# EnnaDelfen/SUHMO

Hardware: AMD Instinct MI355X
Metric: multigrid V-cycles/s (FAS head solve) + GSRB cell-updates/s; achieved HBM GB/s vs peak (higher is better)
Workload: dtype f64; 1 GPU; SHMIP-A head solve, 4096x4096 cells per GPU (square cells of 24.4 m), single AMR level, 64x64 boxes, 6 MG depths, 4+4 GSRB sweeps per depth, 16 bottom (BASELINE north_star: 4096^2 single-level); partition=none

## Files before the change

### suhmo_amd/csrc/suhmo_common.h

```cpp
#pragma once
#include <hip/hip_runtime.h>
#include <cstdio>
#include <cstdlib>
#include <cstring>
#include <utility>
#include <string>
#include <vector>
#include "../../include/suhmo_hip.h"

#define SUHMO_XOFF 16
#define SUHMO_MAXDEPTH 16

struct DV {
    int nx, ny;
    int P;
    int gy;
    int rows;
    int j0, nyg;
    double dx, dy;
    double rdx, rdy;
    double fdx, fdy;
    double alpha, beta;
    int bct[2][2];
    double two_v[2][2];
// ... 112 lines not shown
    int poll_readback;
    size_t scratch_elems;
    suhmo_exchange_fn ex;
    suhmo_allreduce_max_fn ar;
    suhmo_allreduce_fn ar2;
    int (*ard)(void *user, double *dev_values, int n, int op, suhmo_stream_t s);
    void *user;
    int (*ex_begin)(void *user);
    int (*ex_end)(void *user, suhmo_level *L, suhmo_stream_t s);
    long graph_max_cells;
    std::vector<VGraph> vgraphs; int vgraph_seen[4]; hipStream_t gstream;
    suhmo_level *gap; double gap_dt;
    void *rccl;
    int faces_deferred;
    void *ipc; int ipc_owner;
    long agg_min_cells;
    int agg_depth, agg_world, agg_rank;
    suhmo_level *agg;
    int agg_static_stale;
    suhmo_allgather_fn ag; void *ag_user;
    double *agg_send, *agg_recv; size_t agg_cap; long agg_gathers;
    int resout_req, resout_armed, resout_done; const double *resout_rhs; long resout_count;
    int resout_np;
    long frhs_stream, frhs_tile;
    int prof_on;
    std::vector<ProfEv> prof;
    int gsrb_variant;
    long fused_min_cells;
    int bcoef_fused;
    int bcoef_tile_x;
    int fused_nt;
    int fused_restrict;
    int fused_hc;
    int fas_rhs_fused;
    int strips_rhs_local;
    int skip_mask;
    int mask_reported;
    int coarse_mask_ok;
    unsigned mask_epoch, maskflag_epoch;
    int overlap_halo;
    hipStream_t xstream; hipEvent_t xev[2]; long overlapped;
    int tile_strips;
    int tile_chunks;
    int resid_in_relax;
    int fas_rhs_in_relax;
    long tile_max_cells;
    int tile_restrict;
    int tile_order;
    int bottom_solver; long bottom_one_launch_max_cells;
    unsigned long long *bottom_ctr; long bottom_host_iters, bottom_host_solves;
    int gsrb_tile, tile_t, tile_s;
};

void suhmo_set_error(const char *fmt, ...);
struct SuhmoTimer { const char *name; double t0; int mode; explicit SuhmoTimer(const char *n); ~SuhmoTimer(); };
#define SUHMO_TIME(label) SuhmoTimer suhmo_tm_(label)
#define HIPCHK(x) do { hipError_t e_ = (x); if (e_ != hipSuccess) { \
    suhmo_set_error("%s:%d %s -> %s", __FILE__, __LINE__, #x, hipGetErrorString(e_)); return -2; } } while (0)
#define ARG(cond) do { if (!(cond)) { suhmo_set_error("%s:%d bad argument: %s", __FILE__, __LINE__, #cond); return -1; } } while (0)

double *suhmo_field(suhmo_level *L, int depth, int field);
int suhmo_level_create_(suhmo_level_t **out, const suhmo_level_desc_t *desc, bool stub);
void suhmo_level_share_transport(suhmo_level *dst, const suhmo_level *src);
int suhmo_level_materialize_(suhmo_level *L);
void suhmo_fp_changed();
unsigned long suhmo_fp_epoch();
// ... 66 lines not shown
```

### suhmo_amd/csrc/suhmo_gsrb.hip

```cpp
#include "suhmo_hier.h"
#include <type_traits>

template <bool HAS_ALPHA>
__device__ __forceinline__ void d_gsrb_pass_simple(const DV &v, const FP &fp, suhmo_phys_t ph, int pass, int jlo, int jhi,
                                                   const FP *__restrict__ ft = nullptr, const int2 *__restrict__ push = nullptr)
{
    int j = jlo + (int)(blockIdx.y * blockDim.y + threadIdx.y);
    int t = blockIdx.x * blockDim.x + threadIdx.x;
    if (j > jhi) return;
    int i = 2 * t + ((j + v.j0 + pass) & 1);
    if (i >= v.nx) return;
    double *__restrict__ phi = fp.f[SUHMO_F_PHI];
    int idx = cidx(v, i, j);
    double c = phi[idx];
    double e = phiE(v, phi, idx, i, c, false), w = phiW(v, phi, idx, i, c, false);
    double n = phiN(v, phi, idx, j, c, false), s = phiS(v, phi, idx, j, c, false);
    double bxW = fp.f[SUHMO_F_BX][idx], bxE = fp.f[SUHMO_F_BX][idx + 1];
    double byS = fp.f[SUHMO_F_BY][idx], byN = fp.f[SUHMO_F_BY][idx + v.P];
    double nl, dnl;
    nl_terms(ph, c, fp.f[SUHMO_F_B][idx], fp.f[SUHMO_F_PI][idx], fp.f[SUHMO_F_ZB][idx],
             fp.f[SUHMO_F_MASK][idx], nl, dnl);
    double aterm = HAS_ALPHA ? v.alpha * fp.f[SUHMO_F_ACOEF][idx] : v.alpha;
    double lofphi = lofphi_cell(v, aterm, c, e, w, n, s, bxE, bxW, byN, byS, nl);
    double lam = lambda_cell(v, aterm, bxE, bxW, byN, byS);
// ... 202 lines not shown
    const dim3 grd(((m.maxnx + T - 1) / T) * ((m.maxny + T - 1) / T), m.nbox);
    if (has_alpha) hipLaunchKernelGGL((k_gsrb_box_m<true, G, T, S>), grd, dim3(BoxGeom<G, T, S>::NT), 0, st, m.dv, m.fp, (const int2 *)halo, hbase, ph, fsrc, fdst, npass, bc_ghosts);
    else hipLaunchKernelGGL((k_gsrb_box_m<false, G, T, S>), grd, dim3(BoxGeom<G, T, S>::NT), 0, st, m.dv, m.fp, (const int2 *)halo, hbase, ph, fsrc, fdst, npass, bc_ghosts);
}
int suhmo_multi_gsrb_box(const suhmo_multi &m, const suhmo_phys_t &ph, bool has_alpha, const void *halo, const int *hbase, int fsrc, int fdst, int npass, int bc_ghosts, hipStream_t st)
{
    if (m.nbox <= 0) return 0;
    if (npass < 1 || npass > 2 * SUHMO_BOX_HALO) { suhmo_set_error("internal: %d colour passes in one box launch", npass); return -4; }
    if (npass > 4) launch_box<8, 16, 1>(m, ph, has_alpha, halo, hbase, fsrc, fdst, npass, bc_ghosts, st);
    else launch_box<4, 16, 1>(m, ph, has_alpha, halo, hbase, fsrc, fdst, npass, bc_ghosts, st);
    HIPCHK(hipGetLastError());
    return 0;
}

struct FusedGeom {
    int W;
    int Hc;
    int nstrips, nchunks, ntiles;
    int ylo, yhi;
    int jbeg, jend;
    int wrap_y;
    const unsigned *negflag; unsigned mask_epoch;
    int nchl, chunk0, chunk1, edges;
    const double *pc, *pco; int Pc, gyc;
    double *rres, *rphi; int rP, rgy;
    const double *fres; double *frhs, *flphi, *fphiold;
    const double *ortrue; double *ores, *olphi;
    double *onorm;
};

struct RowCoef {
    double rhs[2], B[2], Pi[2], zb[2], mask[2], a[2], byS[2], byN[2];
    double bx0, bx1, bx2;
};
#define CP2(d, s, f) d.f[0] = s.f[0]; d.f[1] = s.f[1]
template <bool HAS_ALPHA>
__device__ __forceinline__ void copy_coef(RowCoef &d, const RowCoef &s)
{
    CP2(d, s, rhs); CP2(d, s, B); CP2(d, s, Pi); CP2(d, s, zb); CP2(d, s, mask);
    if (HAS_ALPHA) { CP2(d, s, a); }
    CP2(d, s, byS); CP2(d, s, byN);
    d.bx0 = s.bx0; d.bx1 = s.bx1; d.bx2 = s.bx2;
}

template <int K, bool HAS_ALPHA, int NT, int RM = 0, bool FRHS = false>
__global__ __launch_bounds__(NT) void k_gsrb_fused(DV v, FP fp, const double *__restrict__ pin,
                                                   double *__restrict__ pout, suhmo_phys_t ph, FusedGeom g)
{
    constexpr bool ROUT = RM == 2, RR = RM != 0;
    static_assert(!(FRHS && (RR || HAS_ALPHA)), "the right-hand side is formed in the plain launch of an alpha = 0 operator");
    constexpr int LW = 2 * NT, R = 2 * K + 3 + (RR ? 1 : 0);
    constexpr int HX = 2 * K + (RR ? 2 : 0), EY = RR ? 1 : 0;
    __shared__ double lds[R * LW];

    int b = blockIdx.x, q = g.ntiles / 8, rem = g.ntiles % 8, xcd = b % 8;
    int tile = xcd * q + (xcd < rem ? xcd : rem) + b / 8;
    int strip = tile / g.nchl, chunk = tile % g.nchl;
    chunk = g.edges ? (chunk < g.chunk0 ? chunk : g.chunk1 + (chunk - g.chunk0)) : g.chunk0 + chunk;

    const int t = threadIdx.x;
    const int c0 = strip * g.W;
    const int xl = 2 * t;
    const int i0 = c0 - HX + xl;
    const bool in_row = xl < g.W + 2 * HX;
    int im = i0;
    if (v.per[0]) { if (im < 0) im += v.nx; else if (im >= v.nx) im -= v.nx; }
    const bool cval = in_row && im >= 0 && im < v.nx;
    const int cend = (c0 + g.W < v.nx) ? c0 + g.W : v.nx;
    const bool own = cval && i0 >= c0 && i0 < cend;

    const int jA = g.jbeg + chunk * g.Hc;
    const int jB = (jA + g.Hc < g.jend) ? jA + g.Hc : g.jend;
    const int jmin = (jA - EY - 2 * K > g.ylo) ? jA - EY - 2 * K : g.ylo;
    const int jmax = (jB - 1 + EY + 2 * K < g.yhi) ? jB - 1 + EY + 2 * K : g.yhi;

    const double *__restrict__ f_rhs = fp.f[SUHMO_F_RHS], *__restrict__ f_B = fp.f[SUHMO_F_B];
    const double *__restrict__ f_Pi = fp.f[SUHMO_F_PI], *__restrict__ f_zb = fp.f[SUHMO_F_ZB];
    const double *__restrict__ f_mask = fp.f[SUHMO_F_MASK], *__restrict__ f_a = fp.f[SUHMO_F_ACOEF];
    const double *__restrict__ f_bx = fp.f[SUHMO_F_BX], *__restrict__ f_by = fp.f[SUHMO_F_BY];

    auto wrapj = [&](int j) { if (g.wrap_y) { if (j < 0) j += v.ny; else if (j >= v.ny) j -= v.ny; } return j; };
    auto ld2 = [&](const double *__restrict__ p, int idx) { return *reinterpret_cast<const double2 *>(p + idx); };

    RowCoef cf0, cf1, cf2, cf3, cf4, cf5;
    double racc = 0.0, raccp = 0.0;
    double nmax = 0.0;
    const bool xbc = !v.per[0] && (c0 - HX <= 0 || c0 + g.W + HX >= v.nx);
    const bool ybc = !v.per[1] && (jmin <= 0 || jmax >= v.ny - 1);
    double2 pnext = make_double2(0.0, 0.0);
    double2 pprev = make_double2(0.0, 0.0);
    const bool usemask = !g.negflag || *g.negflag == g.mask_epoch;

    int sr = 0;
    auto ring = [](int x) { return x < 0 ? x + R : x; };
    for (int r = jmin - 1; r <= jB - 1 + 2 * K + EY; r++) {
        bool lphi = cval && (r + 1 >= jmin) && (r + 1 <= jmax);
        if (lphi) {
            const int jr = wrapj(r + 1);
            pnext = ld2(pin, cidx(v, im, jr));
            if (g.pc) {
                const int ic = ((jr >> 1) + g.gyc) * g.Pc + SUHMO_XOFF + (im >> 1);
                const double corr = 1.0 * g.pc[ic] + (-1.0) * g.pco[ic];
                pnext.x = pnext.x + corr; pnext.y = pnext.y + corr;
            }
        }
        bool lcf = cval && (r >= jmin) && (r <= jmax);
        if (lcf) {
            int idx = cidx(v, im, wrapj(r));
#define LD2(dst, p, ix) { double2 t_ = ld2(p, ix); dst[0] = t_.x; dst[1] = t_.y; }
            LD2(cf0.rhs, (FRHS ? g.fres : f_rhs), idx); LD2(cf0.B, f_B, idx); LD2(cf0.Pi, f_Pi, idx);
            LD2(cf0.zb, f_zb, idx);
            if (usemask) { LD2(cf0.mask, f_mask, idx); } else { cf0.mask[0] = 1.0; cf0.mask[1] = 1.0; }
            if (HAS_ALPHA) LD2(cf0.a, f_a, idx);
            LD2(cf0.byS, f_by, idx); LD2(cf0.byN, f_by, idx + v.P);
            double2 bxp = ld2(f_bx, idx);
            cf0.bx0 = bxp.x; cf0.bx1 = bxp.y; cf0.bx2 = f_bx[idx + 2];
        }
        __syncthreads();

        if constexpr (FRHS) {
            const int jf = r - 1;
            if (cval && jf >= jmin && jf <= jmax) {
                const int s0 = ring(sr - 1), sN = sr;
                const double *row = lds + s0 * LW;
                double lo[2], cc[2];
#pragma unroll
                for (int a = 0; a < 2; a++) {
                    const int x = xl + a, i = im + a;
                    double c = row[x];
                    double w = row[(a == 0 && xl == 0) ? 0 : x - 1], e = row[(a == 1 && xl == LW - 2) ? LW - 1 : x + 1];
                    double n = lds[sN * LW + x], s = a ? pprev.y : pprev.x;
                    if (xbc) {
                        if (i == 0) w = (v.bct[0][0] == 0) ? v.two_v[0][0] - c : c + v.neu[0][0];
                        if (i == v.nx - 1) e = (v.bct[0][1] == 0) ? v.two_v[0][1] - c : c + v.neu[0][1];
                    }
                    if (ybc) {
                        if (jf == 0 && !v.ext[0]) s = (v.bct[1][0] == 0) ? v.two_v[1][0] - c : c + v.neu[1][0];
                        if (jf == v.ny - 1 && !v.ext[1]) n = (v.bct[1][1] == 0) ? v.two_v[1][1] - c : c + v.neu[1][1];
                    }
                    double nl, dnl;
                    nl_terms(ph, c, cf1.B[a], cf1.Pi[a], cf1.zb[a], cf1.mask[a], nl, dnl);
                    const double bxW = a ? cf1.bx1 : cf1.bx0, bxE = a ? cf1.bx2 : cf1.bx1;
                    lo[a] = lofphi_cell(v, v.alpha, c, e, w, n, s, bxE, bxW, cf1.byN[a], cf1.byS[a], nl);
                    cc[a] = c;
                }
                cf1.rhs[0] = 1.0 * cf1.rhs[0] + 1.0 * lo[0]; cf1.rhs[1] = 1.0 * cf1.rhs[1] + 1.0 * lo[1];
                const bool lo_end = v.ext[0] && chunk == 0, hi_end = v.ext[1] && chunk == g.nchunks - 1;
                const int jP0 = lo_end ? jmin : jA, jP1 = hi_end ? jmax + 1 : jB;
                const int jR0 = lo_end ? jmin + 1 : jA, jR1 = hi_end ? jmax : jB;
                if (own && jf >= jP0 && jf < jP1) {
                    const int idx = cidx(v, i0, jf);
                    if (jf >= jR0 && jf < jR1) {
                        *reinterpret_cast<double2 *>(g.flphi + idx) = make_double2(lo[0], lo[1]);
                        *reinterpret_cast<double2 *>(g.frhs + idx) = make_double2(cf1.rhs[0], cf1.rhs[1]);
                    }
                    *reinterpret_cast<double2 *>(g.fphiold + idx) = make_double2(cc[0], cc[1]);
                }
                pprev = make_double2(cc[0], cc[1]);
            }
            __syncthreads();
        }

        auto advance_a = [&](const int m, const RowCoef &q, auto a_tag) {
            constexpr int a = decltype(a_tag)::value;
            const int j = r - m;
            const int x = xl + a, i = im + a;
            const int s0 = ring(sr - m), sN = ring(sr - m + 1), sS = ring(sr - m - 1);
            const double *row = lds + s0 * LW;
            double c = row[x];
            double w = row[(a == 0 && xl == 0) ? 0 : x - 1], e = row[(a == 1 && xl == LW - 2) ? LW - 1 : x + 1];
            double n = lds[sN * LW + x], s = lds[sS * LW + x];
            if (xbc) {
                if (i == 0) w = (v.bct[0][0] == 0) ? v.two_v[0][0] - c : c + v.neu[0][0];
                if (i == v.nx - 1) e = (v.bct[0][1] == 0) ? v.two_v[0][1] - c : c + v.neu[0][1];
            }
            if (ybc) {
                if (j == 0 && !v.ext[0]) s = (v.bct[1][0] == 0) ? v.two_v[1][0] - c : c + v.neu[1][0];
                if (j == v.ny - 1 && !v.ext[1]) n = (v.bct[1][1] == 0) ? v.two_v[1][1] - c : c + v.neu[1][1];
            }
            double nl, dnl;
            nl_terms(ph, c, q.B[a], q.Pi[a], q.zb[a], q.mask[a], nl, dnl);
            const double bxW = a ? q.bx1 : q.bx0, bxE = a ? q.bx2 : q.bx1;
            double aterm = HAS_ALPHA ? v.alpha * q.a[a] : v.alpha;
            double lofphi = lofphi_cell(v, aterm, c, e, w, n, s, bxE, bxW, q.byN[a], q.byS[a], nl);
            double lam = lambda_cell(v, aterm, bxE, bxW, q.byN[a], q.byS[a]);
            double denom = 1.0e-16 + lam + dnl;
            lds[s0 * LW + x] = c + (q.rhs[a] - lofphi) / denom;
        };
        auto advance = [&](const int m, const RowCoef &q) {
            const int j = r - m;
            if (j >= jmin && j <= jmax) {
                const int a = (j + v.j0 + ((m - 1) & 1)) & 1;
                if (a) { if (cval) advance_a(m, q, std::integral_constant<int, 1>()); }
                else   { if (cval) advance_a(m, q, std::integral_constant<int, 0>()); }
            }
        };
        advance(1, cf1);
        __syncthreads();
        advance(2, cf2);
        if constexpr (K >= 2) {
            __syncthreads();
            advance(3, cf3);
            __syncthreads();
            advance(4, cf4);
        }

        if constexpr (RR) {
            const int jr = r - 2 * K - 1;
            if (own && jr >= jA && jr < jB && jr >= 0 && jr < v.ny) {
                const RowCoef &q = (K >= 2) ? cf5 : cf3;
                const int s0 = ring(sr - (2 * K + 1)), sN = ring(sr - 2 * K), sS = ring(sr - (2 * K + 2));
                const double *row = lds + s0 * LW;
                double acc = (jr & 1) ? racc : 0.0, accp = (jr & 1) ? raccp : 0.0;
                double lo2[2] = {0.0, 0.0};
#pragma unroll
                for (int a = 0; a < 2; a++) {
                    const int x = xl + a, i = im + a;
                    double c = row[x], w = row[x - 1], e = row[x + 1];
                    double n = lds[sN * LW + x], s = lds[sS * LW + x];
                    if (xbc) {
                        if (i == 0) w = (v.bct[0][0] == 0) ? v.two_v[0][0] - c : c + v.neu[0][0];
                        if (i == v.nx - 1) e = (v.bct[0][1] == 0) ? v.two_v[0][1] - c : c + v.neu[0][1];
                    }
                    if (ybc) {
                        if (jr == 0 && !v.ext[0]) s = (v.bct[1][0] == 0) ? v.two_v[1][0] - c : c + v.neu[1][0];
                        if (jr == v.ny - 1 && !v.ext[1]) n = (v.bct[1][1] == 0) ? v.two_v[1][1] - c : c + v.neu[1][1];
                    }
                    double nl, dnl;
                    nl_terms(ph, c, q.B[a], q.Pi[a], q.zb[a], q.mask[a], nl, dnl);
                    const double bxW = a ? q.bx1 : q.bx0, bxE = a ? q.bx2 : q.bx1;
                    double aterm = HAS_ALPHA ? v.alpha * q.a[a] : v.alpha;
                    double lofphi = lofphi_cell(v, aterm, c, e, w, n, s, bxE, bxW, q.byN[a], q.byS[a], nl);
                    if constexpr (ROUT) lo2[a] = lofphi;
                    else {
                        acc = acc + (q.rhs[a] - lofphi) / 4.0;
                        accp = accp + c / 4.0;
                    }
                }
                if constexpr (ROUT) {
                    const int idx = cidx(v, i0, jr);
                    const double2 rt = *reinterpret_cast<const double2 *>(g.ortrue + idx);
                    const double r0 = -1.0 * lo2[0] + 1.0 * rt.x, r1 = -1.0 * lo2[1] + 1.0 * rt.y;
                    *reinterpret_cast<double2 *>(g.ores + idx) = make_double2(r0, r1);
                    if (g.olphi) *reinterpret_cast<double2 *>(g.olphi + idx) = make_double2(lo2[0], lo2[1]);
                    nmax = fmax(nmax, fmax(fabs(r0), fabs(r1)));
                } else if (jr & 1) {
                    const int ic = ((jr >> 1) + g.rgy) * g.rP + SUHMO_XOFF + (i0 >> 1);
                    g.rres[ic] = acc; g.rphi[ic] = accp;
                } else { racc = acc; raccp = accp; }
            }
        }
        {
            const int jo = r - 2 * K;
            if (own && jo >= jA && jo < jB) {
                const int so = ring(sr - 2 * K);
                double2 o = make_double2(lds[so * LW + xl], lds[so * LW + xl + 1]);
                *reinterpret_cast<double2 *>(pout + cidx(v, i0, jo)) = o;
            }
        }
        sr = sr + 1 == R ? 0 : sr + 1;
        if (in_row) { lds[sr * LW + xl] = pnext.x; lds[sr * LW + xl + 1] = pnext.y; }
        if constexpr (RR && K >= 2) copy_coef<HAS_ALPHA>(cf5, cf4);
        if constexpr (K >= 2) { copy_coef<HAS_ALPHA>(cf4, cf3); copy_coef<HAS_ALPHA>(cf3, cf2); }
        else if constexpr (RR) copy_coef<HAS_ALPHA>(cf3, cf2);
        copy_coef<HAS_ALPHA>(cf2, cf1);
        copy_coef<HAS_ALPHA>(cf1, cf0);
    }
    if constexpr (ROUT) {
        if (g.onorm) {
            static_assert(!ROUT || NT == 64, "one wave per workgroup");
#pragma unroll
            for (int o = 32; o > 0; o >>= 1) nmax = fmax(nmax, __shfl_xor(nmax, o));
            if (t == 0) g.onorm[strip * g.nchunks + chunk] = nmax;
        }
    }
}

static bool fused_ok(const suhmo_level *L, const Depth &D, int K)
{
    const DV &v = D.v;
    if (v.nx % 2 || v.nx < 64 || v.ny < 4 * K + 4) return false;
    if (v.cfx[0] || v.cfx[1] || L->desc.nx_global > 0) return false;
    if ((v.ext[0] || v.ext[1]) && (v.gy < 2 * K || v.ny < 2 * K)) return false;
    if (v.per[1] && !(v.ext[0] || v.ext[1]) && v.ny < 4 * K) return false;
    return true;
}

template <int K, int NT, int RM = 0>
static int launch_fused(suhmo_level *L, int depth, int ext_rows, hipStream_t st, int part = 0)
{
    constexpr bool RST = RM == 1, RR = RM != 0;
    Depth &D = L->d[depth];
    const DV &v = D.v;
    if (!D.phi_alt) {
        HIPCHK(hipMalloc(&D.phi_alt, D.elems * sizeof(double)));
        HIPCHK(hipMemsetAsync(D.phi_alt, 0, D.elems * sizeof(double), st));
    }
    FusedGeom g;
    constexpr int HX = 2 * K + (RR ? 2 : 0), EY = RR ? 1 : 0;
// ... 48 lines not shown
    g.negflag = nullptr; g.mask_epoch = 0;
    if (L->skip_mask && L->maskflag_epoch && L->maskflag_epoch == L->mask_epoch && (depth == 0 || L->coarse_mask_ok)
        && (L->desc.nx_global == 0)) {
        g.negflag = (const unsigned *)(L->scratch + L->scratch_elems - 1); g.mask_epoch = L->mask_epoch;
    }
    g.rres = g.rphi = nullptr; g.rP = g.rgy = 0;
    if (RST) {
        Depth &C = L->d[depth + 1];
        g.rres = C.fp.f[SUHMO_F_RES]; g.rphi = C.fp.f[SUHMO_F_PHI]; g.rP = C.v.P; g.rgy = C.v.gy;
        C.phi_fresh = 0;
    }
    g.fres = nullptr; g.frhs = g.flphi = g.fphiold = nullptr;
    g.ortrue = nullptr; g.ores = g.olphi = nullptr;
    if (RM == 2) {
        if (v.alpha != 0.0) { suhmo_set_error("internal: residual output on a launch that cannot form it"); return -4; }
        g.ortrue = L->resout_rhs ? L->resout_rhs : D.fp.f[SUHMO_F_RHS];
        g.ores = D.fp.f[SUHMO_F_RES];
        if (L->resout_req & 2) { g.olphi = suhmo_field(L, depth, SUHMO_F_LPHI); if (!g.olphi) return -2; }
        g.onorm = nullptr;
        if ((L->resout_req & 4) && (size_t)g.nstrips * g.nchunks + 4 < L->scratch_elems) { g.onorm = L->scratch + 2; L->resout_np = g.nstrips * g.nchunks; }
        else L->resout_np = 0;
    }
    if (D.rhs_pending) {
        if constexpr (K == 2 && NT == 64 && !RR) {
            if (part || v.alpha != 0.0) { suhmo_set_error("internal: rhs_pending on a launch that cannot form it"); return -4; }
            g.fres = D.fp.f[SUHMO_F_RES]; g.frhs = D.fp.f[SUHMO_F_RHS]; g.flphi = suhmo_field(L, depth, SUHMO_F_LPHI); g.fphiold = suhmo_field(L, depth, SUHMO_F_PHIOLD);
            if (!g.flphi || !g.fphiold) return -2;
            D.rhs_pending = 0; L->frhs_stream++;
            hipLaunchKernelGGL((k_gsrb_fused<2, false, 64, false, true>), dim3(g.ntiles), dim3(NT), 0, st, v, D.fp, pin, D.phi_alt, L->ph, g);
            { std::swap(D.fp.f[SUHMO_F_PHI], D.phi_alt); suhmo_fp_changed(); }
            return 0;
        } else { suhmo_set_error("internal: rhs_pending on a launch that cannot form it"); return -4; }
    }
    if (v.alpha != 0.0)
        hipLaunchKernelGGL((k_gsrb_fused<K, true, NT, false>), dim3(g.ntiles), dim3(NT), 0, st, v, D.fp, pin, D.phi_alt, L->ph, g);
    else
        hipLaunchKernelGGL((k_gsrb_fused<K, false, NT, RM>), dim3(g.ntiles), dim3(NT), 0, st, v, D.fp, pin, D.phi_alt, L->ph, g);
    if (part != 1) { std::swap(D.fp.f[SUHMO_F_PHI], D.phi_alt); suhmo_fp_changed(); }
    return 0;
}

struct TileGeom {
    int ntx, nty;
    const double *pc, *pco; int Pc, gyc;
    double *rres, *rphi; int rP, rgy;
    int frhs;
    int jbeg, jend;
    int chunks;
    int order;
};
struct PairCoef { double rhs0, rhs1, B0, B1, Pi0, Pi1, zb0, zb1, a0, a1, byS0, byS1, byN0, byN1, bx0, bx1, bx2; int mneg; };

template <int T, bool RST> struct TileShape { static constexpr int TX = T, TY = (RST && T == 32) ? 28 : T; };
template <int S, int T, bool RST> struct TileThreads { static constexpr int NT = 256; };
template <int S, int T, bool HAS_ALPHA, bool RST = false, bool CHUNKED = false>
__global__ __launch_bounds__((TileThreads<S, T, RST>::NT)) __attribute__((amdgpu_waves_per_eu((TileThreads<S, T, RST>::NT == 384 ? 3 : 2)))) void k_gsrb_tile(DV v,
    FP fp, const double *__restrict__ pin, double *__restrict__ pout,
                                                   suhmo_phys_t ph, TileGeom g)
{
    constexpr int TX = TileShape<T, RST>::TX, TY = TileShape<T, RST>::TY;
    constexpr int HX = 2 * S + (RST ? 2 : 0), HY = 2 * S + (RST ? 1 : 0);
    constexpr int LX = TX + 2 * HX, LY = TY + 2 * HY, NP = LX / 2, NPAIR = NP * LY;
    constexpr int NT = TileThreads<S, T, RST>::NT, NK = (NPAIR + NT - 1) / NT;
    constexpr int PAD = LX + 2;
    __shared__ double lds_raw[LY * LX + 2 * PAD];
    double *const lds = lds_raw + PAD;
    __shared__ double lq[RST ? TY * TX : 1];
    int tl = blockIdx.x;
    if (g.order) {
// ... 560 lines not shown
```

### suhmo_amd/csrc/suhmo_level.hip

```cpp
#include "suhmo_hier.h"
#include "suhmo_level_int.h"
#include <algorithm>
#include <cstdarg>
#include <cmath>
#include <initializer_list>

static thread_local char g_err[512] = "";
void suhmo_set_error(const char *fmt, ...)
{
    va_list ap; va_start(ap, fmt); vsnprintf(g_err, sizeof(g_err), fmt, ap); va_end(ap);
}
extern "C" const char *suhmo_last_error(void) { return g_err; }
#include <atomic>
#include <chrono>
#include <map>
#include <mutex>
namespace {
std::atomic<int> g_timer_mode{-1};
std::mutex g_timer_mu;
struct TimerRec { long count = 0; double total = 0.0; };
std::map<std::string, TimerRec> g_timers;
inline double now_s() { return std::chrono::duration<double>(std::chrono::steady_clock::now().time_since_epoch()).count(); }
inline int timer_mode()
{
// ... 108 lines not shown
{
    ARG(out && desc);
    ARG(desc->nx >= 2 && desc->ny >= 2 && desc->dx > 0 && desc->dy > 0);
    ARG(desc->ny_global >= desc->ny && desc->j0 >= 0 && desc->j0 + desc->ny <= desc->ny_global);
    ARG(desc->i0 >= 0 && (desc->nx_global == 0 ? desc->i0 == 0 : desc->i0 + desc->nx <= desc->nx_global));
    ARG(desc->i0 % 2 == 0);
    ARG(desc->patch_ny == 0 || (desc->nx_global > 0 && desc->patch_j0 <= desc->j0 && desc->j0 + desc->ny <= desc->patch_j0 + desc->patch_ny));
    ARG((long)(desc->nx + 64) * (long)(desc->ny + 2 * (desc->halo_rows < 1 ? 1 : desc->halo_rows)) < (1L << 31));
    int ndev = 0;
    HIPCHK(hipGetDeviceCount(&ndev));
    if (ndev <= 0) { suhmo_set_error("no HIP device: the product path has no CPU fallback"); return -3; }
    ARG(desc->device >= 0 && desc->device < ndev);
    HIPCHK(hipSetDevice(desc->device));
    suhmo_level *L = new suhmo_level();
    L->desc = *desc; L->ph = desc->phys; L->device = desc->device;
    L->ex = nullptr; L->ar = nullptr; L->ar2 = nullptr; L->ard = nullptr; L->user = nullptr; L->ex_begin = nullptr; L->ex_end = nullptr; L->rccl = nullptr;
        L->ipc = nullptr; L->ipc_owner = 0; L->faces_deferred = 0; L->gap = nullptr; L->gap_dt = 0.0; L->prof_on = 0; L->gsrb_variant = -1; L->fused_hc = 0;
    L->bcoef_fused = 1;
    L->bcoef_tile_x = 62;
    L->fused_nt = 64;
    L->fused_restrict = 1;
    L->gsrb_tile = 1; L->tile_t = 0; L->tile_s = 4;
    L->tile_max_cells = 3000000;
    L->fas_rhs_in_relax = 3;
    L->tile_chunks = 1;
    L->tile_order = 2; L->tile_restrict = 0;
    L->tile_strips = 1;
    L->overlap_halo = 1; L->xstream = nullptr; L->xev[0] = L->xev[1] = nullptr; L->overlapped = 0;
    L->strips_rhs_local = 1;
    L->fas_rhs_fused = 1;
    L->agg_min_cells = 100000; L->agg_depth = 0; L->agg_world = 1; L->agg_rank = 0; L->agg = nullptr; L->ag = nullptr; L->ag_user = nullptr;
    L->agg_send = L->agg_recv = nullptr; L->agg_cap = 0; L->agg_gathers = 0; L->agg_static_stale = 0;
    L->frhs_stream = L->frhs_tile = 0;
    L->resout_np = 0;
    L->resout_req = L->resout_armed = L->resout_done = 0; L->resout_rhs = nullptr; L->resout_count = 0; L->resid_in_relax = 1;
    L->graph_max_cells = 1500000; L->gstream = nullptr; memset(L->vgraph_seen, 0, sizeof(L->vgraph_seen));
    L->fused_min_cells = 1000000;
    L->skip_mask = 1; L->poll_readback = 1;
    L->bottom_solver = 0; L->bottom_one_launch_max_cells = 16384;
    L->bottom_ctr = nullptr; L->bottom_host_iters = L->bottom_host_solves = 0;
    {
        struct IntKnob { const char *env; int suhmo_level::*field; };
        struct LongKnob { const char *env; long suhmo_level::*field; };
        static const IntKnob ints[] = {
            {"SUHMO_GSRB_VARIANT", &suhmo_level::gsrb_variant}, {"SUHMO_FUSED_HC", &suhmo_level::fused_hc}, {"SUHMO_BCOEF_FUSED", &suhmo_level::bcoef_fused},
            {"SUHMO_BCOEF_TILE_X", &suhmo_level::bcoef_tile_x}, {"SUHMO_FUSED_NT", &suhmo_level::fused_nt}, {"SUHMO_OVERLAP_HALO", &suhmo_level::overlap_halo},
            {"SUHMO_STRIPS_RHS_LOCAL", &suhmo_level::strips_rhs_local}, {"SUHMO_FAS_RHS_FUSED", &suhmo_level::fas_rhs_fused},
            {"SUHMO_RESID_IN_RELAX", &suhmo_level::resid_in_relax}, {"SUHMO_TILE_STRIPS", &suhmo_level::tile_strips}, {"SUHMO_TILE_CHUNKS", &suhmo_level::tile_chunks},
            {"SUHMO_TILE_RESTRICT", &suhmo_level::tile_restrict}, {"SUHMO_TILE_ORDER", &suhmo_level::tile_order}, {"SUHMO_FAS_RHS_IN_RELAX", &suhmo_level::fas_rhs_in_relax},
            {"SUHMO_TILE_S", &suhmo_level::tile_s}, {"SUHMO_GSRB_TILE", &suhmo_level::gsrb_tile}, {"SUHMO_TILE_T", &suhmo_level::tile_t},
            {"SUHMO_FUSED_RESTRICT", &suhmo_level::fused_restrict}, {"SUHMO_SKIP_MASK", &suhmo_level::skip_mask}, {"SUHMO_POLL_READBACK", &suhmo_level::poll_readback}};
        static const LongKnob longs[] = {
            {"SUHMO_AGG_MIN_CELLS", &suhmo_level::agg_min_cells}, {"SUHMO_TILE_MAX_CELLS", &suhmo_level::tile_max_cells},
            {"SUHMO_GRAPH_MAX_CELLS", &suhmo_level::graph_max_cells}, {"SUHMO_FUSED_MIN_CELLS", &suhmo_level::fused_min_cells},
            {"SUHMO_BOTTOM_ONE_LAUNCH_MAX_CELLS", &suhmo_level::bottom_one_launch_max_cells}};
        for (const IntKnob &k : ints) if (const char *e = getenv(k.env)) L->*(k.field) = atoi(e);
        for (const LongKnob &k : longs) if (const char *e = getenv(k.env)) L->*(k.field) = atol(e);
        L->fas_rhs_fused = L->fas_rhs_fused != 0;
        if (L->tile_order < 0 || L->tile_order > 2) L->tile_order = 0;
        if (L->tile_t != 16 && L->tile_t != 32) L->tile_t = 0;
    }
    if (desc->boxes && desc->nbox > 0) {
        L->boxes.assign(desc->boxes, desc->boxes + 4 * (size_t)desc->nbox);
    } else {
        int mb = desc->max_box > 0 ? desc->max_box : 64;
        for (int bj = 0; bj * mb < desc->ny; bj++)
            for (int bi = 0; bi * mb < desc->nx; bi++) {
                int lo0 = desc->i0 + bi * mb, lo1 = desc->j0 + bj * mb;
                int hi0 = std::min(lo0 + mb, desc->i0 + desc->nx) - 1, hi1 = std::min(lo1 + mb, desc->j0 + desc->ny) - 1;
                int b[4] = {lo0, lo1, hi0, hi1};
                L->boxes.insert(L->boxes.end(), b, b + 4);
            }
    }
    L->desc.boxes = nullptr;
    L->desc.nbox = (int)(L->boxes.size() / 4);
    {
        long cells = 0;
        for (size_t k = 0; k < L->boxes.size(); k += 4) {
            const int *b = &L->boxes[k];
            if (b[0] < desc->i0 || b[2] >= desc->i0 + desc->nx || b[1] < desc->j0 || b[3] >= desc->j0 + desc->ny || b[0] > b[2] || b[1] > b[3]) {
                suhmo_set_error("box %zu outside the strip", k / 4); delete L; return -1;
            }
            cells += (long)(b[2] - b[0] + 1) * (b[3] - b[1] + 1);
        }
        if (cells != (long)desc->nx * desc->ny) { suhmo_set_error("boxes do not tile the level"); delete L; return -1; }
    }
    L->ndepth = 1;
    for (int dep = 1; dep < SUHMO_MAXDEPTH; dep++) {
        if (!boxes_coarsenable(L->boxes, (1 << dep) * 2)) break;
        if ((desc->j0 % (1 << dep)) || (desc->ny_global % (1 << dep))) break;
        if ((desc->i0 % (2 << dep)) || (desc->nx_global % (1 << dep))) break;
        L->ndepth = dep + 1;
    }
// ... 63 lines not shown
    for (int dep = 0; dep < L->ndepth; dep++) make_dv(L->d[dep].v, L->desc, dep);
    suhmo_level_drop_graphs(L);
    return 0;
}
extern "C" int suhmo_level_set_alpha_beta(suhmo_level_t *L, double alpha, double beta)
{
    ARG(L);
    L->desc.alpha = alpha; L->desc.beta = beta;
    if (L->agg) { int rc = suhmo_level_set_alpha_beta(L->agg, alpha, beta); if (rc) return rc; }
    return remake_views(L);
}
extern "C" int suhmo_level_set_bc(suhmo_level_t *L, const suhmo_bc_t *bc)
{
    ARG(L && bc);
    for (int d = 0; d < 2; d++)
        if ((bc->periodic[d] != 0) != (L->desc.bc.periodic[d] != 0)) { suhmo_set_error("setBC cannot change the periodicity of the domain"); return -1; }
    for (int d = 0; d < 2; d++) for (int s = 0; s < 2; s++) ARG(bc->type[d][s] == 0 || bc->type[d][s] == 1);
    L->desc.bc = *bc;
    if (L->agg) { int rc = suhmo_level_set_bc(L->agg, bc); if (rc) return rc; }
    return remake_views(L);
}

static long *option_slot_long(suhmo_level *L, const char *key)
{
    if (!strcmp(key, "fused_min_cells")) return &L->fused_min_cells;
    if (!strcmp(key, "tile_max_cells")) return &L->tile_max_cells;
    if (!strcmp(key, "graph_max_cells")) return &L->graph_max_cells;
    if (!strcmp(key, "agg_min_cells")) return &L->agg_min_cells;
    return nullptr;
}
static int *option_slot_int(suhmo_level *L, const char *key)
{
    static const struct { const char *k; int suhmo_level::*m; } tab[] = {
        {"gsrb_variant", &suhmo_level::gsrb_variant}, {"fused_hc", &suhmo_level::fused_hc}, {"bcoef_fused", &suhmo_level::bcoef_fused}, {"bcoef_tile_x", &suhmo_level::bcoef_tile_x},
        {"fused_nt", &suhmo_level::fused_nt}, {"fused_restrict", &suhmo_level::fused_restrict}, {"strips_rhs_local", &suhmo_level::strips_rhs_local},
        {"tile_strips", &suhmo_level::tile_strips}, {"overlap_halo", &suhmo_level::overlap_halo}, {"skip_mask", &suhmo_level::skip_mask}, {"tile_chunks",
            &suhmo_level::tile_chunks}, {"tile_order", &suhmo_level::tile_order}, {"tile_restrict", &suhmo_level::tile_restrict}, {"fas_rhs_in_relax",
            &suhmo_level::fas_rhs_in_relax}, {"resid_in_relax", &suhmo_level::resid_in_relax}, {"fas_rhs_fused", &suhmo_level::fas_rhs_fused},
        {"tile_s", &suhmo_level::tile_s}, {"gsrb_tile", &suhmo_level::gsrb_tile}, {"tile_t", &suhmo_level::tile_t}, {"poll_readback", &suhmo_level::poll_readback}};
    for (const auto &e : tab) if (!strcmp(key, e.k)) return &(L->*(e.m));
    return nullptr;
}
extern "C" int suhmo_level_set_option(suhmo_level_t *L, const char *key, long value)
{
    ARG(L && key);
    if (!strcmp(key, "bottom_solver")) {
        if (value != 0 && value != 1) { suhmo_set_error("bottom_solver: 0 (bottom relaxes only) or 1 (RelaxSolver)"); return -1; }
        return suhmo_bottom_configure(L, (int)value, L->bottom_one_launch_max_cells);
    }
    if (!strcmp(key, "bottom_one_launch_max_cells")) {
        if (value < 0) { suhmo_set_error("bottom_one_launch_max_cells: >= 0"); return -1; }
        return suhmo_bottom_configure(L, L->bottom_solver, value);
    }
    if (long *p = option_slot_long(L, key)) {
        *p = value; suhmo_level_drop_graphs(L);
        if (!strcmp(key, "agg_min_cells")) return suhmo_agg_setup(L);
        return 0;
    }
    if (int *p = option_slot_int(L, key)) {
        if (!strcmp(key, "tile_t") && value != 0 && value != 16 && value != 32) { suhmo_set_error("tile_t: 0 (by size), 16 or 32"); return -1; }
        if (!strcmp(key, "fused_nt") && value != 64 && value != 256) { suhmo_set_error("fused_nt: 64 or 256"); return -1; }
        if (!strcmp(key, "poll_readback") && value && !L->hscratch_dev) { suhmo_set_error("poll_readback: no device address of the host slot"); return -1; }
        *p = (int)value; suhmo_level_drop_graphs(L); return 0;
    }
    suhmo_set_error("unknown option '%s'", key);
    return -1;
}
extern "C" int suhmo_level_get_option(const suhmo_level_t *L, const char *key, long *value)
{
    ARG(L && key && value);
    if (long *p = option_slot_long(const_cast<suhmo_level *>(L), key)) { *value = *p; return 0; }
    if (int *p = option_slot_int(const_cast<suhmo_level *>(L), key)) { *value = *p; return 0; }
    if (!strcmp(key, "overlapped_launches")) { *value = L->overlapped; return 0; }
    if (!strcmp(key, "agg_gathers")) { *value = L->agg_gathers; return 0; }
    if (!strcmp(key, "rhs_in_streaming_launches")) { *value = L->frhs_stream; return 0; }
    if (!strcmp(key, "rhs_in_tile_launches")) { *value = L->frhs_tile; return 0; }
    if (!strcmp(key, "residual_in_relax_launches")) { *value = L->resout_count; return 0; }
    if (!strcmp(key, "bottom_solver")) { *value = L->bottom_solver; return 0; }
    if (!strcmp(key, "bottom_one_launch_max_cells")) { *value = L->bottom_one_launch_max_cells; return 0; }
    if (!strcmp(key, "bottom_solver_iterations")) { *value = suhmo_bottom_counter(L, 0); return 0; }
    if (!strcmp(key, "bottom_solves_one_launch")) { *value = suhmo_bottom_counter(L, 1); return 0; }
    if (!strcmp(key, "bottom_solves_host_loop")) { *value = suhmo_bottom_counter(L, 2); return 0; }
    suhmo_set_error("unknown option '%s'", key);
    return -1;
}

extern "C" int suhmo_level_num_depths(const suhmo_level_t *L) { return L ? L->ndepth : -1; }
extern "C" int suhmo_level_synchronize(suhmo_level_t *L, suhmo_stream_t s)
{
    ARG(L);
    HIPCHK(hipStreamSynchronize((hipStream_t)s));
    return 0;
}
extern "C" int suhmo_level_set_hooks(suhmo_level_t *L, suhmo_exchange_fn ex, suhmo_allreduce_max_fn ar, void *user)
{
    ARG(L);
    L->ex = ex; L->ar = ar; L->ar2 = nullptr; L->ard = nullptr; L->user = user; L->ex_begin = nullptr; L->ex_end = nullptr;
    return 0;
}
void suhmo_level_share_transport(suhmo_level *dst, const suhmo_level *src)
{
    dst->ex = src->ex; dst->ar = src->ar; dst->ar2 = src->ar2; dst->ard = src->ard; dst->user = src->user;
    dst->ex_begin = src->ex_begin; dst->ex_end = src->ex_end; dst->ipc = src->ipc;
}
extern "C" int suhmo_level_set_allgather(suhmo_level_t *L, suhmo_allgather_fn fn, void *user)
{
    ARG(L);
    HIPCHK(hipSetDevice(L->device));
    L->ag = fn; L->ag_user = user;
// ... 228 lines not shown
```

Measured before the change: 487.0 V-cycles/s.

## Add opt-in two-row load prefetch to fused GSRB and trim coefficient registers

Restructures the fused GSRB row loop into issue/step phases so an optional variant can keep loads for two rows in flight, raising memory-level parallelism for the plain alpha=0, K=2, 64-thread launch. The default path also changes: the mask is kept as a sign bitfield, the south face coefficient is reused from the previous row's north face instead of reloaded, and the coarse correction is applied at store time. These changes cut global loads and register pressure, but the mask now enters as ±1, and the two-row path raises register use and is gated behind an option.

Measured after the change: 493.3 V-cycles/s, median of 6. 1.01x the previous value.

```diff
diff --git a/suhmo_amd/csrc/suhmo_common.h b/suhmo_amd/csrc/suhmo_common.h
--- a/suhmo_amd/csrc/suhmo_common.h
+++ b/suhmo_amd/csrc/suhmo_common.h
@@ -168,6 +168,8 @@
     int fused_nt;
     int fused_restrict;
     int fused_hc;
+    int fused_prefetch;
+    long prefetch2_count;
     int fas_rhs_fused;
     int strips_rhs_local;
     int skip_mask;
diff --git a/suhmo_amd/csrc/suhmo_gsrb.hip b/suhmo_amd/csrc/suhmo_gsrb.hip
--- a/suhmo_amd/csrc/suhmo_gsrb.hip
+++ b/suhmo_amd/csrc/suhmo_gsrb.hip
@@ -258,23 +258,35 @@
 struct RowCoef {
     double rhs[2], B[2], Pi[2], zb[2], mask[2], a[2], byS[2], byN[2];
     double bx0, bx1, bx2;
+    int mneg;
 };
 #define CP2(d, s, f) d.f[0] = s.f[0]; d.f[1] = s.f[1]
 template <bool HAS_ALPHA>
 __device__ __forceinline__ void copy_coef(RowCoef &d, const RowCoef &s)
 {
-    CP2(d, s, rhs); CP2(d, s, B); CP2(d, s, Pi); CP2(d, s, zb); CP2(d, s, mask);
+    CP2(d, s, rhs); CP2(d, s, B); CP2(d, s, Pi); CP2(d, s, zb); d.mneg = s.mneg;
     if (HAS_ALPHA) { CP2(d, s, a); }
     CP2(d, s, byS); CP2(d, s, byN);
     d.bx0 = s.bx0; d.bx1 = s.bx1; d.bx2 = s.bx2;
 }
-
-template <int K, bool HAS_ALPHA, int NT, int RM = 0, bool FRHS = false>
-__global__ __launch_bounds__(NT) void k_gsrb_fused(DV v, FP fp, const double *__restrict__ pin,
+template <bool HAS_ALPHA>
+__device__ __forceinline__ void enter_coef(RowCoef &d, const RowCoef &ld, const RowCoef &below)
+{
+    CP2(d, ld, rhs); CP2(d, ld, B); CP2(d, ld, Pi); CP2(d, ld, zb);
+    d.mneg = (ld.mask[0] < 0.0 ? 1 : 0) | (ld.mask[1] < 0.0 ? 2 : 0);
+    if (HAS_ALPHA) { CP2(d, ld, a); }
+    d.byS[0] = below.byN[0]; d.byS[1] = below.byN[1];
+    CP2(d, ld, byN);
+    d.bx0 = ld.bx0; d.bx1 = ld.bx1; d.bx2 = ld.bx2;
+}
+
+template <int K, bool HAS_ALPHA, int NT, int RM = 0, bool FRHS = false, int PF = 1>
+__global__ __launch_bounds__(NT) __attribute__((amdgpu_waves_per_eu(PF == 2 ? 2 : 1))) void k_gsrb_fused(DV v, FP fp, const double *__restrict__ pin,
                                                    double *__restrict__ pout, suhmo_phys_t ph, FusedGeom g)
 {
     constexpr bool ROUT = RM == 2, RR = RM != 0;
     static_assert(!(FRHS && (RR || HAS_ALPHA)), "the right-hand side is formed in the plain launch of an alpha = 0 operator");
+    static_assert(PF == 1 || (PF == 2 && !RR && !FRHS && !HAS_ALPHA), "two rows in flight: the plain launch only");
     constexpr int LW = 2 * NT, R = 2 * K + 3 + (RR ? 1 : 0);
     constexpr int HX = 2 * K + (RR ? 2 : 0), EY = RR ? 1 : 0;
     __shared__ double lds[R * LW];
@@ -308,40 +320,42 @@
     auto wrapj = [&](int j) { if (g.wrap_y) { if (j < 0) j += v.ny; else if (j >= v.ny) j -= v.ny; } return j; };
     auto ld2 = [&](const double *__restrict__ p, int idx) { return *reinterpret_cast<const double2 *>(p + idx); };
 
-    RowCoef cf0, cf1, cf2, cf3, cf4, cf5;
+    RowCoef cf0, cfN, cf1, cf2, cf3, cf4, cf5;
     double racc = 0.0, raccp = 0.0;
     double nmax = 0.0;
     const bool xbc = !v.per[0] && (c0 - HX <= 0 || c0 + g.W + HX >= v.nx);
     const bool ybc = !v.per[1] && (jmin <= 0 || jmax >= v.ny - 1);
-    double2 pnext = make_double2(0.0, 0.0);
+    double2 pnext = make_double2(0.0, 0.0), pnextN = make_double2(0.0, 0.0);
+    double2 pcor = make_double2(0.0, 0.0), pcorN = make_double2(0.0, 0.0);
     double2 pprev = make_double2(0.0, 0.0);
     const bool usemask = !g.negflag || *g.negflag == g.mask_epoch;
 
     int sr = 0;
     auto ring = [](int x) { return x < 0 ? x + R : x; };
-    for (int r = jmin - 1; r <= jB - 1 + 2 * K + EY; r++) {
-        bool lphi = cval && (r + 1 >= jmin) && (r + 1 <= jmax);
-        if (lphi) {
-            const int jr = wrapj(r + 1);
-            pnext = ld2(pin, cidx(v, im, jr));
-            if (g.pc) {
+#define LD2(dst, p, ix) { double2 t_ = ld2(p, ix); dst[0] = t_.x; dst[1] = t_.y; }
+    auto issue = [&](const int r, RowCoef &ct, double2 &pt, double2 &qt) __attribute__((always_inline)) {
+        const int jp = r + PF, jc = r + PF - 1;
+        if (cval && jp >= jmin && jp <= jmax) {
+            const int jr = wrapj(jp);
+            pt = ld2(pin, cidx(v, im, jr));
+            if (PF == 1 && g.pc) {
                 const int ic = ((jr >> 1) + g.gyc) * g.Pc + SUHMO_XOFF + (im >> 1);
-                const double corr = 1.0 * g.pc[ic] + (-1.0) * g.pco[ic];
-                pnext.x = pnext.x + corr; pnext.y = pnext.y + corr;
-            }
-        }
-        bool lcf = cval && (r >= jmin) && (r <= jmax);
-        if (lcf) {
-            int idx = cidx(v, im, wrapj(r));
-#define LD2(dst, p, ix) { double2 t_ = ld2(p, ix); dst[0] = t_.x; dst[1] = t_.y; }
-            LD2(cf0.rhs, (FRHS ? g.fres : f_rhs), idx); LD2(cf0.B, f_B, idx); LD2(cf0.Pi, f_Pi, idx);
-            LD2(cf0.zb, f_zb, idx);
-            if (usemask) { LD2(cf0.mask, f_mask, idx); } else { cf0.mask[0] = 1.0; cf0.mask[1] = 1.0; }
-            if (HAS_ALPHA) LD2(cf0.a, f_a, idx);
-            LD2(cf0.byS, f_by, idx); LD2(cf0.byN, f_by, idx + v.P);
+                qt.x = g.pc[ic]; qt.y = g.pco[ic];
+            }
+        }
+        if (cval && jc >= jmin && jc <= jmax) {
+            int idx = cidx(v, im, wrapj(jc));
+            LD2(ct.rhs, (FRHS ? g.fres : f_rhs), idx); LD2(ct.B, f_B, idx); LD2(ct.Pi, f_Pi, idx);
+            LD2(ct.zb, f_zb, idx);
+            if (usemask) { LD2(ct.mask, f_mask, idx); } else { ct.mask[0] = 1.0; ct.mask[1] = 1.0; }
+            if (HAS_ALPHA) LD2(ct.a, f_a, idx);
+            LD2(ct.byN, f_by, idx + v.P);
             double2 bxp = ld2(f_bx, idx);
-            cf0.bx0 = bxp.x; cf0.bx1 = bxp.y; cf0.bx2 = f_bx[idx + 2];
-        }
+            ct.bx0 = bxp.x; ct.bx1 = bxp.y; ct.bx2 = f_bx[idx + 2];
+        }
+    };
+    auto step = [&](const int r, RowCoef &ct, double2 &pt, double2 &qt, RowCoef &cc, double2 &pc, double2 &qc) __attribute__((always_inline)) {
+        issue(r, ct, pt, qt);
         __syncthreads();
 
         if constexpr (FRHS) {
@@ -365,7 +379,7 @@
                         if (jf == v.ny - 1 && !v.ext[1]) n = (v.bct[1][1] == 0) ? v.two_v[1][1] - c : c + v.neu[1][1];
                     }
                     double nl, dnl;
-                    nl_terms(ph, c, cf1.B[a], cf1.Pi[a], cf1.zb[a], cf1.mask[a], nl, dnl);
+                    nl_terms(ph, c, cf1.B[a], cf1.Pi[a], cf1.zb[a], (cf1.mneg >> a) & 1 ? -1.0 : 1.0, nl, dnl);
                     const double bxW = a ? cf1.bx1 : cf1.bx0, bxE = a ? cf1.bx2 : cf1.bx1;
                     lo[a] = lofphi_cell(v, v.alpha, c, e, w, n, s, bxE, bxW, cf1.byN[a], cf1.byS[a], nl);
                     cc[a] = c;
@@ -405,7 +419,7 @@
                 if (j == v.ny - 1 && !v.ext[1]) n = (v.bct[1][1] == 0) ? v.two_v[1][1] - c : c + v.neu[1][1];
             }
             double nl, dnl;
-            nl_terms(ph, c, q.B[a], q.Pi[a], q.zb[a], q.mask[a], nl, dnl);
+            nl_terms(ph, c, q.B[a], q.Pi[a], q.zb[a], (q.mneg >> a) & 1 ? -1.0 : 1.0, nl, dnl);
             const double bxW = a ? q.bx1 : q.bx0, bxE = a ? q.bx2 : q.bx1;
             double aterm = HAS_ALPHA ? v.alpha * q.a[a] : v.alpha;
             double lofphi = lofphi_cell(v, aterm, c, e, w, n, s, bxE, bxW, q.byN[a], q.byS[a], nl);
@@ -453,7 +467,7 @@
                         if (jr == v.ny - 1 && !v.ext[1]) n = (v.bct[1][1] == 0) ? v.two_v[1][1] - c : c + v.neu[1][1];
                     }
                     double nl, dnl;
-                    nl_terms(ph, c, q.B[a], q.Pi[a], q.zb[a], q.mask[a], nl, dnl);
+                    nl_terms(ph, c, q.B[a], q.Pi[a], q.zb[a], (q.mneg >> a) & 1 ? -1.0 : 1.0, nl, dnl);
                     const double bxW = a ? q.bx1 : q.bx0, bxE = a ? q.bx2 : q.bx1;
                     double aterm = HAS_ALPHA ? v.alpha * q.a[a] : v.alpha;
                     double lofphi = lofphi_cell(v, aterm, c, e, w, n, s, bxE, bxW, q.byN[a], q.byS[a], nl);
@@ -485,12 +499,31 @@
             }
         }
         sr = sr + 1 == R ? 0 : sr + 1;
-        if (in_row) { lds[sr * LW + xl] = pnext.x; lds[sr * LW + xl + 1] = pnext.y; }
+        if (in_row) {
+            double2 pe = pc;
+            if (PF == 1 && g.pc) {
+                const double corr = 1.0 * qc.x + (-1.0) * qc.y;
+                pe.x = pe.x + corr; pe.y = pe.y + corr;
+            }
+            lds[sr * LW + xl] = pe.x; lds[sr * LW + xl + 1] = pe.y;
+        }
         if constexpr (RR && K >= 2) copy_coef<HAS_ALPHA>(cf5, cf4);
         if constexpr (K >= 2) { copy_coef<HAS_ALPHA>(cf4, cf3); copy_coef<HAS_ALPHA>(cf3, cf2); }
         else if constexpr (RR) copy_coef<HAS_ALPHA>(cf3, cf2);
         copy_coef<HAS_ALPHA>(cf2, cf1);
-        copy_coef<HAS_ALPHA>(cf1, cf0);
+        enter_coef<HAS_ALPHA>(cf1, cc, cf2);
+        if (g.wrap_y && (r == 0 || r == v.ny) && cval && r >= jmin && r <= jmax) LD2(cf1.byS, f_by, cidx(v, im, wrapj(r)));
+    };
+    const int rend = jB - 1 + 2 * K + EY;
+    if (cval && jmin <= jmax) LD2(cf0.byN, f_by, cidx(v, im, wrapj(jmin)));
+    if constexpr (PF == 1) {
+        for (int r = jmin - 1; r <= rend; r++) step(r, cf0, pnext, pcor, cf0, pnext, pcor);
+    } else {
+        issue(jmin - 2, cf0, pnext, pcor);
+        for (int r = jmin - 1; r <= rend; r += 2) {
+            step(r, cfN, pnextN, pcorN, cf0, pnext, pcor);
+            if (r + 1 <= rend) step(r + 1, cf0, pnext, pcor, cfN, pnextN, pcorN);
+        }
     }
     if constexpr (ROUT) {
         if (g.onorm) {
@@ -605,9 +638,16 @@
             return 0;
         } else { suhmo_set_error("internal: rhs_pending on a launch that cannot form it"); return -4; }
     }
+    bool two_rows = false;
+    if constexpr (K == 2 && NT == 64 && !RR) two_rows = L->fused_prefetch == 2 && v.alpha == 0.0 && !g.pc;
     if (v.alpha != 0.0)
         hipLaunchKernelGGL((k_gsrb_fused<K, true, NT, false>), dim3(g.ntiles), dim3(NT), 0, st, v, D.fp, pin, D.phi_alt, L->ph, g);
-    else
+    else if (two_rows) {
+        if constexpr (K == 2 && NT == 64 && !RR) {
+            hipLaunchKernelGGL((k_gsrb_fused<2, false, 64, 0, false, 2>), dim3(g.ntiles), dim3(NT), 0, st, v, D.fp, pin, D.phi_alt, L->ph, g);
+            L->prefetch2_count++;
+        }
+    } else
         hipLaunchKernelGGL((k_gsrb_fused<K, false, NT, RM>), dim3(g.ntiles), dim3(NT), 0, st, v, D.fp, pin, D.phi_alt, L->ph, g);
     if (part != 1) { std::swap(D.fp.f[SUHMO_F_PHI], D.phi_alt); suhmo_fp_changed(); }
     return 0;
diff --git a/suhmo_amd/csrc/suhmo_level.hip b/suhmo_amd/csrc/suhmo_level.hip
--- a/suhmo_amd/csrc/suhmo_level.hip
+++ b/suhmo_amd/csrc/suhmo_level.hip
@@ -164,6 +164,7 @@
     L->agg_min_cells = 100000; L->agg_depth = 0; L->agg_world = 1; L->agg_rank = 0; L->agg = nullptr; L->ag = nullptr; L->ag_user = nullptr;
     L->agg_send = L->agg_recv = nullptr; L->agg_cap = 0; L->agg_gathers = 0; L->agg_static_stale = 0;
     L->frhs_stream = L->frhs_tile = 0;
+    L->fused_prefetch = 1; L->prefetch2_count = 0;
     L->resout_np = 0;
     L->resout_req = L->resout_armed = L->resout_done = 0; L->resout_rhs = nullptr; L->resout_count = 0; L->resid_in_relax = 1;
     L->graph_max_cells = 1500000; L->gstream = nullptr; memset(L->vgraph_seen, 0, sizeof(L->vgraph_seen));
@@ -175,7 +176,7 @@
         struct IntKnob { const char *env; int suhmo_level::*field; };
         struct LongKnob { const char *env; long suhmo_level::*field; };
         static const IntKnob ints[] = {
-            {"SUHMO_GSRB_VARIANT", &suhmo_level::gsrb_variant}, {"SUHMO_FUSED_HC", &suhmo_level::fused_hc}, {"SUHMO_BCOEF_FUSED", &suhmo_level::bcoef_fused},
+            {"SUHMO_GSRB_VARIANT", &suhmo_level::gsrb_variant}, {"SUHMO_FUSED_HC", &suhmo_level::fused_hc}, {"SUHMO_FUSED_PREFETCH", &suhmo_level::fused_prefetch}, {"SUHMO_BCOEF_FUSED", &suhmo_level::bcoef_fused},
             {"SUHMO_BCOEF_TILE_X", &suhmo_level::bcoef_tile_x}, {"SUHMO_FUSED_NT", &suhmo_level::fused_nt}, {"SUHMO_OVERLAP_HALO", &suhmo_level::overlap_halo},
             {"SUHMO_STRIPS_RHS_LOCAL", &suhmo_level::strips_rhs_local}, {"SUHMO_FAS_RHS_FUSED", &suhmo_level::fas_rhs_fused},
             {"SUHMO_RESID_IN_RELAX", &suhmo_level::resid_in_relax}, {"SUHMO_TILE_STRIPS", &suhmo_level::tile_strips}, {"SUHMO_TILE_CHUNKS", &suhmo_level::tile_chunks},
@@ -191,6 +192,7 @@
         L->fas_rhs_fused = L->fas_rhs_fused != 0;
         if (L->tile_order < 0 || L->tile_order > 2) L->tile_order = 0;
         if (L->tile_t != 16 && L->tile_t != 32) L->tile_t = 0;
+        if (L->fused_prefetch != 2) L->fused_prefetch = 1;
     }
     if (desc->boxes && desc->nbox > 0) {
         L->boxes.assign(desc->boxes, desc->boxes + 4 * (size_t)desc->nbox);
@@ -320,7 +322,7 @@
 static int *option_slot_int(suhmo_level *L, const char *key)
 {
     static const struct { const char *k; int suhmo_level::*m; } tab[] = {
-        {"gsrb_variant", &suhmo_level::gsrb_variant}, {"fused_hc", &suhmo_level::fused_hc}, {"bcoef_fused", &suhmo_level::bcoef_fused}, {"bcoef_tile_x", &suhmo_level::bcoef_tile_x},
+        {"gsrb_variant", &suhmo_level::gsrb_variant}, {"fused_hc", &suhmo_level::fused_hc}, {"fused_prefetch", &suhmo_level::fused_prefetch}, {"bcoef_fused", &suhmo_level::bcoef_fused}, {"bcoef_tile_x", &suhmo_level::bcoef_tile_x},
         {"fused_nt", &suhmo_level::fused_nt}, {"fused_restrict", &suhmo_level::fused_restrict}, {"strips_rhs_local", &suhmo_level::strips_rhs_local},
         {"tile_strips", &suhmo_level::tile_strips}, {"overlap_halo", &suhmo_level::overlap_halo}, {"skip_mask", &suhmo_level::skip_mask}, {"tile_chunks",
             &suhmo_level::tile_chunks}, {"tile_order", &suhmo_level::tile_order}, {"tile_restrict", &suhmo_level::tile_restrict}, {"fas_rhs_in_relax",
@@ -348,6 +350,7 @@
     if (int *p = option_slot_int(L, key)) {
         if (!strcmp(key, "tile_t") && value != 0 && value != 16 && value != 32) { suhmo_set_error("tile_t: 0 (by size), 16 or 32"); return -1; }
         if (!strcmp(key, "fused_nt") && value != 64 && value != 256) { suhmo_set_error("fused_nt: 64 or 256"); return -1; }
+        if (!strcmp(key, "fused_prefetch") && value != 1 && value != 2) { suhmo_set_error("fused_prefetch: 1 or 2 rows of loads in flight"); return -1; }
         if (!strcmp(key, "poll_readback") && value && !L->hscratch_dev) { suhmo_set_error("poll_readback: no device address of the host slot"); return -1; }
         *p = (int)value; suhmo_level_drop_graphs(L); return 0;
     }
@@ -363,6 +366,7 @@
     if (!strcmp(key, "agg_gathers")) { *value = L->agg_gathers; return 0; }
     if (!strcmp(key, "rhs_in_streaming_launches")) { *value = L->frhs_stream; return 0; }
     if (!strcmp(key, "rhs_in_tile_launches")) { *value = L->frhs_tile; return 0; }
+    if (!strcmp(key, "two_row_prefetch_launches")) { *value = L->prefetch2_count; return 0; }
     if (!strcmp(key, "residual_in_relax_launches")) { *value = L->resout_count; return 0; }
     if (!strcmp(key, "bottom_solver")) { *value = L->bottom_solver; return 0; }
     if (!strcmp(key, "bottom_one_launch_max_cells")) { *value = L->bottom_one_launch_max_cells; return 0; }
```
